# Aster32/GAN-DANet

Measured on AMD Instinct MI355X. Metric: train samples/sec (G+D step) on 256x256 tiles, higher is better.
Workload: dtype bf16; 1 GPU; full G+D train step, 8ch 256x256 -> 1024x1024 tiles, batch 32/GPU (global 32), perceptual=on, SSIM evaluated, AdamW x2; survey_config=3, per_gpu_batch=32, global_batch=32, tile=256, parallelism=dp1

## Files before the change

### gan-danet_amd/csrc/pam.hip

```cpp
#include <stdlib.h>
#include <type_traits>

#include "pam_common.h"
#include "../../include/gandanet.h"

namespace {

using namespace pam;

__device__ __forceinline__ f32x16_t mfma_bf16(bf16x8_t a, bf16x8_t b, f32x16_t c) { return mfma16<false>(a, b, c); }
__device__ __forceinline__ bf16x8_t pack_frag(const f32x16_t& a, int s) { return pam::pack_frag<false>(a, s); }

constexpr int F_KLD = 40;

constexpr int D_KROWCH = 5;

template <int CT, int NW, int KT, bool ONES, bool F16>
__global__ __launch_bounds__(NW * 64, 2) void pam_fwd_dma_kernel(const unsigned short* __restrict__ qt,
                                                            const unsigned short* __restrict__ kt,
                                                            const unsigned short* __restrict__ v, int N, int Npad, int C,
                                                            const float* __restrict__ gamma, const float* __restrict__ x,
                                                            long x_bs, float* __restrict__ out, long out_bs,
                                                            float* __restrict__ o_attn, float* __restrict__ lse,
                                                            const float* __restrict__ k_sqmax,
                                                            const float* __restrict__ mshift, int* __restrict__ redo) {
    if (redo && !mshift && redo[blockIdx.y * gridDim.x + blockIdx.x] == 0) return;
    constexpr int CP = CT * 32;
    constexpr int NSUB = KT / 32;
    constexpr int VROWCH = KT / 8 + 1;
    constexpr int VLD = KT + 8;
    constexpr int KCH = KT * D_KROWCH;
    constexpr int NCH = KCH + CP * VROWCH;
    constexpr int NPIECE = (NCH + 63) / 64;
    constexpr int PPW = (NPIECE + NW - 1) / NW;
    constexpr int TILE = NPIECE * 64 * 8;
    __shared__ __attribute__((aligned(16))) unsigned short ring[2 * TILE];

    const int tid = threadIdx.x, lane = tid & 63, wave = tid >> 6;
    const int r = lane & 31, h = lane >> 5;
    const int b = blockIdx.y;
    const int q0 = blockIdx.x * (NW * 32) + wave * 32;
    const unsigned short* ktb = kt + (long)b * Npad * 32;
    const unsigned short* vb = v + (long)b * CP * Npad;

    bf16x8_t qf[2];
#pragma unroll
    for (int s = 0; s < 2; ++s)
        qf[s] = *reinterpret_cast<const bf16x8_t*>(qt + ((long)b * Npad + q0 + r) * 32 + s * 16 + 8 * h);

    static_assert(KCH % 64 == 0, "a DMA piece must be all-K or all-V");
    unsigned int voff[PPW];
#pragma unroll
    for (int i = 0; i < PPW; ++i) {
        const int piece = wave + NW * i;
        const int c = piece * 64 + lane;
        if (piece * 64 < KCH) {
            const int row = c / D_KROWCH, part = c - row * D_KROWCH;
            voff[i] = (unsigned int)(row * 32 + (part < 4 ? part : 3) * 8) * 2u;
        } else {
            const int c2 = (c < NCH ? c : NCH - 1) - KCH;
            const int row = c2 / VROWCH, part = c2 - row * VROWCH;
            voff[i] = ((unsigned int)row * (unsigned int)Npad + (unsigned int)(part < KT / 8 ? part : KT / 8 - 1) * 8u) * 2u;
        }
    }
    auto dma_tile = [&](int t, int slot) {
        const char* kbase = reinterpret_cast<const char*>(ktb + (long)t * (KT * 32));
        const char* vbase = reinterpret_cast<const char*>(vb + (long)t * KT);
#pragma unroll
        for (int i = 0; i < PPW; ++i) {
            const int piece = wave + NW * i;
            if (piece < NPIECE && piece * 64 + lane < NCH) {
                unsigned short* dst = ring + slot * TILE + piece * 512;
                const char* base = piece * 64 < KCH ? kbase : vbase;
                __builtin_amdgcn_global_load_lds((const __attribute__((address_space(1))) void*)(base + voff[i]),
                                                 (__attribute__((address_space(3))) void*)dst, 16, 0, 0);
            }
        }
    };

    f32x16_t o[CT];
#pragma unroll
    for (int ct = 0; ct < CT; ++ct)
#pragma unroll
        for (int e = 0; e < 16; ++e) o[ct][e] = 0.f;
    float m = 0.f, l = 0.f;
    const int nkt = (N + KT - 1) / KT;

    dma_tile(0, 0);
    auto sweep = [&](auto nm) {
    constexpr bool NOMAX = decltype(nm)::value;
    for (int t = 0; t < nkt; ++t) {
        asm volatile("s_waitcnt vmcnt(0)" ::: "memory");
        __syncthreads();
        if (t + 1 < nkt) dma_tile(t + 1, (t + 1) & 1);
        const unsigned short* Ks = ring + (t & 1) * TILE;
        const unsigned short* Vs = Ks + KCH * 8;

        f32x16_t sacc[NSUB];
#pragma unroll
        for (int sub = 0; sub < NSUB; ++sub) {
#pragma unroll
            for (int e = 0; e < 16; ++e) sacc[sub][e] = 0.f;
#pragma unroll
            for (int s = 0; s < 2; ++s) {
                const bf16x8_t kf = *reinterpret_cast<const bf16x8_t*>(Ks + (sub * 32 + r) * F_KLD + s * 16 + 8 * h);
                sacc[sub] = mfma16<F16>(kf, qf[s], sacc[sub]);
            }
        }
        if ((t + 1) * KT > N) {
#pragma unroll
            for (int sub = 0; sub < NSUB; ++sub)
#pragma unroll
                for (int e = 0; e < 16; ++e)
                    if ((t * KT + sub * 32 + acc_row(e, h)) >= N) sacc[sub][e] = -1e30f;
        }
        float mloc = sacc[0][0];
        if constexpr (!NOMAX) {
#pragma unroll
            for (int sub = 0; sub < NSUB; ++sub)
#pragma unroll
                for (int e = 0; e < 16; ++e) mloc = fmaxf(mloc, sacc[sub][e]);
            mloc = fmaxf(mloc, __shfl_xor(mloc, 32, 64));
        }
        float lsum = 0.f;
        bf16x8_t pf[NSUB][2];
        if (!NOMAX && (t == 0 || __any(mloc > 0.f))) {
            const float want = m + (t == 0 ? mloc : fmaxf(mloc, 0.f));
            float m_new;
            unsigned short m_neg16;
            if constexpr (F16) {
                _Float16 hm = (_Float16)want;
                unsigned short hb = __builtin_bit_cast(unsigned short, hm);
                if ((float)hm < want) hb = (hb & 0x8000u) ? (unsigned short)(hb - 1) : (unsigned short)(hb + 1);
                m_new = (float)__builtin_bit_cast(_Float16, hb);
                m_neg16 = hb ^ 0x8000u;
            } else {
                const unsigned int wb = __builtin_bit_cast(unsigned int, want);
                m_new = __builtin_bit_cast(float, want > 0.f ? (wb + 0xFFFFu) & 0xFFFF0000u : wb & 0xFFFF0000u);
                m_neg16 = (unsigned short)(__builtin_bit_cast(unsigned int, -m_new) >> 16);
            }
            const float shift = m_new - m;
            if (t != 0) {
                const float alpha = gd_exp2_fast(-shift);
                l *= alpha;
#pragma unroll
                for (int ct = 0; ct < CT; ++ct)
#pragma unroll
                    for (int e = 0; e < 16; ++e) o[ct][e] *= alpha;
            }
            m = m_new;
            if (h) qf[1][7] = (short)m_neg16;
#pragma unroll
            for (int sub = 0; sub < NSUB; ++sub) {
#pragma unroll
                for (int e = 0; e < 16; ++e) {
                    sacc[sub][e] = gd_exp2_fast(sacc[sub][e] - shift);
                    if (!ONES) lsum += sacc[sub][e];
                }
                pf[sub][0] = pam::pack_frag<F16>(sacc[sub], 0);
                pf[sub][1] = pam::pack_frag<F16>(sacc[sub], 1);
            }
        } else {
#pragma unroll
            for (int sub = 0; sub < NSUB; ++sub) {
#pragma unroll
                for (int e = 0; e < 16; ++e) {
                    sacc[sub][e] = gd_exp2_fast(sacc[sub][e]);
                    if (!ONES) lsum += sacc[sub][e];
                }
                pf[sub][0] = pam::pack_frag<F16>(sacc[sub], 0);
                pf[sub][1] = pam::pack_frag<F16>(sacc[sub], 1);
            }
        }
        if (!ONES) {
            lsum += __shfl_xor(lsum, 32, 64);
            l += lsum;
        }

#pragma unroll
        for (int ks = 0; ks < 2 * NSUB; ++ks) {
            const int sub = ks >> 1, s2 = ks & 1;
            bf16x8_t vf[CT];
#pragma unroll
            for (int ct = 0; ct < CT; ++ct)
                vf[ct] = *reinterpret_cast<const bf16x8_t*>(Vs + (ct * 32 + r) * VLD + sub * 32 + s2 * 16 + 8 * h);
            __builtin_amdgcn_sched_group_barrier(0x100, CT, 0);
#pragma unroll
            for (int ct = 0; ct < CT; ++ct) o[ct] = mfma16<F16>(vf[ct], pf[sub][s2], o[ct]);
            __builtin_amdgcn_sched_group_barrier(0x008, CT, 0);
        }
    }
    };
    bool nomax = false;
    if (mshift) {
        float mv = mshift[(long)b * Npad + q0 + r];
        m = mv;
        if (h) qf[1][7] = (short)(__builtin_bit_cast(unsigned int, -mv) >> 16);
        nomax = true;
    } else if (k_sqmax) {
        float q2 = 0.f;
#pragma unroll
        for (int s = 0; s < 2; ++s)
#pragma unroll
            for (int e = 0; e < 8; ++e) {
                const float qv = F16 ? (float)__builtin_bit_cast(_Float16, (unsigned short)qf[s][e]) : gd_bf2f((unsigned short)qf[s][e]);
                q2 = fmaf(qv, qv, q2);
            }
        q2 += __shfl_xor(q2, 32, 64);
        const float bound = sqrtf(q2 * k_sqmax[b]) * 1.0001f;
        nomax = __syncthreads_and(bound <= (F16 ? 13.f : 60.f)) != 0;
    }
    if (nomax) sweep(std::true_type{});
    else sweep(std::false_type{});

    if (ONES) l = __shfl(o[CT - 1][15], r + 32, 64);
    if (mshift) {
        const bool bad = !(l > 1e-30f && l < 1e30f) && (q0 + r) < N;
        if (__syncthreads_or(bad) && tid == 0) redo[blockIdx.y * gridDim.x + blockIdx.x] = 1;
    }
    const int qi = q0 + r;
    if (qi < N) {
        const float inv_l = 1.f / l;
        const float g = *gamma;
#pragma unroll
        for (int ct = 0; ct < CT; ++ct)
#pragma unroll
            for (int e = 0; e < 16; ++e) {
                const int c = ct * 32 + acc_row(e, h);
                if (c < C) {
                    const float val = o[ct][e] * inv_l;
                    o_attn[((long)b * C + c) * N + qi] = val;
                    out[(long)b * out_bs + (long)c * N + qi] = fmaf(g, val, x[(long)b * x_bs + (long)c * N + qi]);
                }
            }
        if (h == 0) lse[(long)b * N + qi] = (m + log2f(l)) * LN2;
    }
}


template <int NS, bool F16>
__global__ __launch_bounds__(256) void pam_row_shift_kernel(const unsigned short* __restrict__ qt,
                                                           const unsigned short* __restrict__ kt, int N, int Npad,
                                                           float* __restrict__ mshift) {
    __shared__ __attribute__((aligned(16))) unsigned short ks[NS * 32];
    const int b = blockIdx.y, tid = threadIdx.x;
    const long nb = (long)b * Npad;
    const int stride = N / NS > 0 ? N / NS : 1;
    for (int c = tid; c < NS * 4; c += 256) {
        const int j = c >> 2, part = c & 3;
        const long key = (long)j * stride < N ? (long)j * stride : (long)N - 1;
        *reinterpret_cast<u32x4_t*>(ks + j * 32 + part * 8) = *reinterpret_cast<const u32x4_t*>(kt + (nb + key) * 32 + part * 8);
    }
    __syncthreads();
    const int i = blockIdx.x * 256 + tid;
    if (i >= Npad) return;
    float q[32];
    {
        const u32x4_t* qp = reinterpret_cast<const u32x4_t*>(qt + (nb + i) * 32);
#pragma unroll
        for (int c = 0; c < 4; ++c) {
            const u32x4_t w = qp[c];
#pragma unroll
            for (int e = 0; e < 4; ++e) {
                q[c * 8 + 2 * e] = pam::unpack_lo<F16>(w[e]);
                q[c * 8 + 2 * e + 1] = pam::unpack_hi<F16>(w[e]);
            }
        }
        q[31] = 0.f;
    }
    float best = -3.0e38f;
    for (int j = 0; j < NS; ++j) {
        const u32x4_t* kp = reinterpret_cast<const u32x4_t*>(ks + j * 32);
        float d = 0.f;
#pragma unroll
        for (int c = 0; c < 4; ++c) {
            const u32x4_t w = kp[c];
#pragma unroll
            for (int e = 0; e < 4; ++e) {
                d = fmaf(q[c * 8 + 2 * e], pam::unpack_lo<F16>(w[e]), d);
                d = fmaf(q[c * 8 + 2 * e + 1], pam::unpack_hi<F16>(w[e]), d);
            }
        }
        best = fmaxf(best, d);
    }
    const unsigned int wb = __builtin_bit_cast(unsigned int, best);
    const float up = __builtin_bit_cast(float, best > 0.f ? (wb + 0xFFFFu) & 0xFFFF0000u : wb & 0xFFFF0000u);
    mshift[nb + i] = up;
}

template <int CT, bool DQ, int NW = 4>
__global__ __launch_bounds__(NW * 64, NW == 4 ? 2 : 1) void pam_bwd_dkv3_kernel(
    const unsigned short* __restrict__ qt, const unsigned short* __restrict__ kt, const unsigned short* __restrict__ kn,
    const unsigned short* __restrict__ vt, const unsigned short* __restrict__ dot_, const float* __restrict__ lse,
    const float* __restrict__ delta, int N, int Npad, float* __restrict__ dkn, float* __restrict__ dv,
    unsigned short* __restrict__ dq_part) {
    constexpr int CP = CT * 32;
    constexpr int NT = NW * 64, KEYS = NW * 32;
    constexpr int DLD = CP + 8;
    constexpr int NCHUNK = 128 + 128 * CT;
    constexpr int NPRE = (NCHUNK + NT - 1) / NT;
    constexpr bool RAGGED = (NCHUNK % NT) != 0;
    __shared__ __attribute__((aligned(16))) unsigned short Vls[KEYS * DLD];
    __shared__ __attribute__((aligned(16))) unsigned short Qs[32 * B_QLD];
    constexpr int DOLD = CP + 32;
    __shared__ __attribute__((aligned(16))) unsigned short dOs[32 * DOLD];
    __shared__ float Ls[32], Ds[32];
    constexpr int XLD = 36;
    __shared__ __attribute__((aligned(16))) unsigned short Xs[DQ ? NW * 32 * XLD : 8];

    const int tid = threadIdx.x, lane = tid & 63, wave = tid >> 6;
    const int r = lane & 31, h = lane >> 5;
    const int b = blockIdx.y;
    const int j0 = blockIdx.x * KEYS + wave * 32;
    const long nb = (long)b * Npad;

    bf16x8_t kfB[2];
#pragma unroll
    for (int s = 0; s < 2; ++s) kfB[s] = *reinterpret_cast<const bf16x8_t*>(kt + (nb + j0 + r) * 32 + s * 16 + 8 * h);
    bf16x8_t knA[2];
    if (DQ) {
#pragma unroll
        for (int s = 0; s < 2; ++s)
            knA[s] = *reinterpret_cast<const bf16x8_t*>(kn + ((long)b * 32 + r) * Npad + j0 + s * 16 + 8 * h);
    }
    unsigned short* Xw = Xs + (DQ ? wave * 32 * XLD : 0);
    unsigned short* part = DQ ? dq_part + ((long)b * (Npad / KEYS) + blockIdx.x) * Npad * 32 : nullptr;
    {
        const unsigned short* vsrc = vt + (nb + (long)blockIdx.x * KEYS) * CP;
        for (int c = tid; c < KEYS * (CP / 8); c += NT) {
            const int row = c / (CP / 8), ch = c - row * (CP / 8);
            *reinterpret_cast<u32x4_t*>(Vls + row * DLD + ch * 8) =
                *reinterpret_cast<const u32x4_t*>(vsrc + (long)row * CP + ch * 8);
        }
    }

    f32x16_t dvacc[CT], dkacc;
#pragma unroll
    for (int e = 0; e < 16; ++e) dkacc[e] = 0.f;
#pragma unroll
    for (int ct = 0; ct < CT; ++ct)
#pragma unroll
        for (int e = 0; e < 16; ++e) dvacc[ct][e] = 0.f;

    const bool key_ok = (j0 + r) < N;
// ... 453 lines not shown
```

### gan-danet_amd/csrc/conv3x3.hip

```cpp
#include "common.h"
#include "tile_mma.h"
#include "../../include/gandanet.h"

namespace {

using gd::acc_row;
using gd::bf16x8_native_t;
typedef unsigned int u32x4_t __attribute__((ext_vector_type(4)));

constexpr int TW = 32;
constexpr int PW = TW + 2;
constexpr int CK = 32;
constexpr int LD = CK + 8;

__global__ void pack_w_kernel(const float* __restrict__ a, long a_sm, long a_sc, long a_st, int M, int Ck, int flip,
                              int BM, int nchunks, unsigned short* __restrict__ wp, long total) {
    for (long i = (long)blockIdx.x * blockDim.x + threadIdx.x; i < total; i += (long)gridDim.x * blockDim.x) {
        const int cc = (int)(i % CK);
        long t = i / CK;
        const int mm = (int)(t % BM);
        t /= BM;
        const int tap = (int)(t % 9);
        t /= 9;
        const int chunk = (int)(t % nchunks);
// ... 602 lines not shown
            const long pbase = (((long)b * a.H + Y) * a.W + X) * (a.split ? 3 * a.K : a.K);
#pragma unroll
            for (int g = 0; g < 4; ++g) {
                const int m = mt * BM + wm * 32 + 8 * g + 4 * h;
                if (m >= a.K) continue;
                float v[4];
#pragma unroll
                for (int k = 0; k < 4; ++k) v[k] = acc[c][j][4 * g + k];
                if (a.act) {
                    const uint2 mk = *reinterpret_cast<const uint2*>(a.act + pbase + m);
                    if (!((mk.x & 0x7FFFu) && !(mk.x & 0x8000u))) v[0] *= a.slope;
                    if (!((mk.x >> 16) & 0x7FFFu) || (mk.x >> 31)) v[1] *= a.slope;
                    if (!((mk.y & 0x7FFFu) && !(mk.y & 0x8000u))) v[2] *= a.slope;
                    if (!((mk.y >> 16) & 0x7FFFu) || (mk.y >> 31)) v[3] *= a.slope;
                }
                uint2 o;
                if (a.split) {
                    uint2 lo;
                    gd_split_bf2(v[0], v[1], o.x, lo.x);
                    gd_split_bf2(v[2], v[3], o.y, lo.y);
                    *reinterpret_cast<uint2*>(a.dx + pbase + a.K + m) = lo;
                    *reinterpret_cast<uint2*>(a.dx + pbase + 2 * a.K + m) = o;
                } else {
                    o.x = gd_pack_bf2(v[0], v[1]);
                    o.y = gd_pack_bf2(v[2], v[3]);
                }
                *reinterpret_cast<uint2*>(a.dx + pbase + m) = o;
            }
        }
    }
}

}

extern "C" int gd_conv3x3_nhwc_pack(const float* w, int Cout, int Cin, int transposed, void* ws, size_t ws_bytes,
                                    void* stream) {
    GD_CHECK_ARG(w && ws && Cout > 0 && Cin > 0 && transposed >= 0 && transposed <= 2, "gd_conv3x3_nhwc_pack: bad arguments");
    const int M = transposed ? Cin : Cout, K = transposed ? Cout : Cin;
    GD_CHECK_ARG(ws_bytes >= gd_conv3x3_ws_bytes(M, K), "gd_conv3x3_nhwc_pack: workspace too small");
    const int bm = transposed == 2 ? 64 : pick_bm(M, K);
    const int mtiles = (M + bm - 1) / bm, nchunks = (K + CK - 1) / CK;
    const long total = (long)mtiles * nchunks * 9 * bm * CK;
    int blocks = (int)((total + 255) / 256);
    if (blocks > 2048) blocks = 2048;
    const long sm = transposed ? 9 : (long)Cin * 9, sc = transposed ? (long)Cin * 9 : 9;
    hipLaunchKernelGGL(pack_w_kernel, dim3(blocks), dim3(256), 0, (hipStream_t)stream, w, sm, sc, 1L, M, K,
                       transposed == 1 ? 1 : 0, bm, nchunks, (unsigned short*)ws, total);
    GD_LAUNCH_CHECK();
    return 0;
}

static int nhwc_conv_launch(const void* x, const void* wpack, const float* bias, const void* mask, const void* res,
                            void* y, int B, int H, int W, int K, int M, int stride, int act, float slope, void* stream,
                            float* y32 = nullptr, long y32_bs = 0, int osplit = 0) {
    NhwcConvArgs a;
    static const int epi_env = getenv("GD_NHWC_EPI_LDS") ? atoi(getenv("GD_NHWC_EPI_LDS")) : 1;
    a.y32 = y32; a.y32_bs = y32_bs; a.osplit = osplit; a.epi_lds = epi_env;
    a.x = (const unsigned short*)x; a.wp = (const unsigned short*)wpack; a.bias = bias;
    a.mask = (const unsigned short*)mask; a.res = (const unsigned short*)res; a.y = (unsigned short*)y;
    a.H = H; a.W = W; a.K = K; a.M = M; a.act = act; a.slope = slope;
    a.Ho = (H - 1) / stride + 1; a.Wo = (W - 1) / stride + 1;
    const int bm = pick_bm(M, K);
    const int mtiles = (M + bm - 1) / bm;
    a.nchunks = (K + CK - 1) / CK;
    a.tiles_x = (a.Wo + TW - 1) / TW;
    const int th = stride == 1 ? 8 : 4;
    const int tiles_y = (a.Ho + th - 1) / th;
    dim3 grid(a.tiles_x * tiles_y, mtiles, B);
    hipStream_t s = (hipStream_t)stream;
    if (!a.y32 && a.epi_lds) {
        if (stride == 1) {
            if (bm == 64) hipLaunchKernelGGL((conv3x3_nhwc_kernel<64, 1, 1>), grid, dim3(256), 0, s, a);
            else hipLaunchKernelGGL((conv3x3_nhwc_kernel<128, 1, 1>), grid, dim3(256), 0, s, a);
        } else {
            if (bm == 64) hipLaunchKernelGGL((conv3x3_nhwc_kernel<64, 2, 1>), grid, dim3(256), 0, s, a);
            else hipLaunchKernelGGL((conv3x3_nhwc_kernel<128, 2, 1>), grid, dim3(256), 0, s, a);
        }
    } else if (stride == 1) {
        if (bm == 64) hipLaunchKernelGGL((conv3x3_nhwc_kernel<64, 1>), grid, dim3(256), 0, s, a);
        else hipLaunchKernelGGL((conv3x3_nhwc_kernel<128, 1>), grid, dim3(256), 0, s, a);
    } else {
        if (bm == 64) hipLaunchKernelGGL((conv3x3_nhwc_kernel<64, 2>), grid, dim3(256), 0, s, a);
        else hipLaunchKernelGGL((conv3x3_nhwc_kernel<128, 2>), grid, dim3(256), 0, s, a);
    }
    GD_LAUNCH_CHECK();
    return 0;
}

extern "C" int gd_conv3x3_nhwc(const void* x, const void* wpack, const float* bias, const void* mask, const void* res,
                               void* y, int B, int H, int W, int K, int M, int relu, int split, void* stream) {
    GD_CHECK_ARG(x && wpack && y, "gd_conv3x3_nhwc: null pointer");
    GD_CHECK_ARG(B > 0 && B <= 65535 && H > 0 && W > 0 && K > 0 && M > 0 && K % 8 == 0 && M % 8 == 0,
                 "gd_conv3x3_nhwc: channel counts must be multiples of 8");
    GD_CHECK_ARG((long)H * W * K < (1L << 31) && (long)H * W * M * (split ? 3 : 1) < (1L << 31), "gd_conv3x3_nhwc: image too large");
    return nhwc_conv_launch(x, wpack, bias, mask, res, y, B, H, W, K, M, 1, relu ? 1 : 0, 0.f, stream, nullptr, 0, split ? 1 : 0);
}

extern "C" int gd_conv3x3_nhwc_f32out(const void* x, const void* wpack, const float* bias, float* y32, long y_bs, int B, int H,
                                      int W, int K, int M, int relu, void* stream) {
    GD_CHECK_ARG(x && wpack && y32, "gd_conv3x3_nhwc_f32out: null pointer");
    GD_CHECK_ARG(B > 0 && B <= 65535 && H > 0 && W > 0 && K > 0 && M > 0 && K % 8 == 0 && M % 4 == 0 && y_bs >= (long)M * H * W,
                 "gd_conv3x3_nhwc_f32out: K must be a multiple of 8, M of 4");
    GD_CHECK_ARG((long)H * W * K < (1L << 31), "gd_conv3x3_nhwc_f32out: image too large");
    return nhwc_conv_launch(x, wpack, bias, nullptr, nullptr, nullptr, B, H, W, K, M, 1, relu ? 1 : 0, 0.f, stream, y32, y_bs);
}

extern "C" int gd_conv3x3_nhwc_s2(const void* x, const void* wpack, const float* bias, void* y, int B, int H, int W, int K,
                                  int M, int act, float slope, int split, void* stream) {
    GD_CHECK_ARG(x && wpack && y, "gd_conv3x3_nhwc_s2: null pointer");
    GD_CHECK_ARG(B > 0 && B <= 65535 && H > 0 && W > 0 && K > 0 && M > 0 && K % 8 == 0 && M % 8 == 0 && act >= 0 && act <= 2,
                 "gd_conv3x3_nhwc_s2: channel counts must be multiples of 8, act in 0..2");
    GD_CHECK_ARG((long)H * W * K < (1L << 31) && (long)H * W * M * (split ? 3 : 1) < (1L << 31), "gd_conv3x3_nhwc_s2: image too large");
    return nhwc_conv_launch(x, wpack, bias, nullptr, nullptr, y, B, H, W, K, M, 2, act, slope, stream, nullptr, 0, split ? 1 : 0);
}

extern "C" int gd_conv3x3_nhwc_s2_dgrad(const void* dy, const void* wpack_t, const void* act_out, float slope, void* dx,
                                        int B, int H, int W, int K, int M, int split, void* stream) {
    GD_CHECK_ARG(dy && wpack_t && dx, "gd_conv3x3_nhwc_s2_dgrad: null pointer");
    GD_CHECK_ARG(B > 0 && B <= 65535 && H > 0 && W > 0 && K > 0 && M > 0 && K % 8 == 0 && M % 8 == 0,
                 "gd_conv3x3_nhwc_s2_dgrad: channel counts must be multiples of 8");
    GD_CHECK_ARG((long)H * W * K * (split ? 3 : 1) < (1L << 31) && (long)H * W * M < (1L << 31), "gd_conv3x3_nhwc_s2_dgrad: image too large");
    NhwcDgrad2Args a;
    a.split = split ? 1 : 0;
    a.dy = (const unsigned short*)dy; a.wp = (const unsigned short*)wpack_t; a.act = (const unsigned short*)act_out;
    a.dx = (unsigned short*)dx; a.H = H; a.W = W; a.K = K; a.M = M; a.slope = slope;
    a.Ho = (H - 1) / 2 + 1; a.Wo = (W - 1) / 2 + 1;
    a.nchunks = (M + CK - 1) / CK;
    a.tiles_x = (a.Wo + TW - 1) / TW;
    const int tiles_y = (a.Ho + 3) / 4;
    dim3 grid(a.tiles_x * tiles_y, (K + 63) / 64, B);
    hipLaunchKernelGGL(conv3x3_nhwc_dgrad2_kernel, grid, dim3(256), 0, (hipStream_t)stream, a);
    GD_LAUNCH_CHECK();
    return 0;
}

namespace {

typedef short s16x4_t __attribute__((ext_vector_type(4)));
constexpr int WTH = 4;
constexpr int WPH = WTH + 2;
constexpr int WNPIX = WPH * PW;
constexpr int DYLD = WTH * TW + 8;

struct WgradArgs {
    const unsigned short* dy16;
    const float* dy; long dy_bs;
    const float* x; long x_bs;
    const unsigned short* x16; int x16_ld;
    const float* in_scale; const float* in_shift; int in_relu;
    float* dw;
    float* part;
    int B, M, Ck, H, W, Ho, Wo;
    int tiles_x, tiles_y, tiles_per_split;
};
typedef float f32x4u_t __attribute__((ext_vector_type(4), aligned(4)));

__device__ __forceinline__ s16x4_t lds_tr_read(const unsigned short* p) {
    return __builtin_amdgcn_ds_read_tr16_b64_v4i16((__attribute__((address_space(3))) s16x4_t*)p);
}

#ifndef GD_WGRAD_PIPED_MINW
#define GD_WGRAD_PIPED_MINW 1
#endif
template <int NW, int S, bool CS, bool PIPED = false, bool ORD = false>
__global__ __launch_bounds__(NW * 64, PIPED ? GD_WGRAD_PIPED_MINW : 2) void conv3x3_wgrad_kernel(const WgradArgs a) {
    constexpr int BM = CS ? 32 : 32 * NW, NT = 64 * NW, NCH = CS ? NW : 1;
    constexpr int PHk = S * (WTH - 1) + 3, PWk = S * (TW - 1) + 3, NPIXk = PHk * PWk;
    __shared__ __attribute__((aligned(16))) unsigned short dys[BM * DYLD];
    __shared__ __attribute__((aligned(16))) unsigned short patch[NCH * NPIXk * LD];

    const int tid = threadIdx.x, lane = tid & 63, wave = tid >> 6;
    const int r = lane & 31, h = lane >> 5;
    const int c0 = blockIdx.x * CK * NCH;
    const int m0 = blockIdx.y * BM;
    const long HW = (long)a.H * a.W;
    const long HWo = (long)a.Ho * a.Wo;
    const int ntiles = a.B * a.tiles_y * a.tiles_x;
    const int t_begin = blockIdx.z * a.tiles_per_split;
    const int t_end = min(ntiles, t_begin + a.tiles_per_split);

    f32x16_t acc[9];
#pragma unroll
    for (int t = 0; t < 9; ++t)
#pragma unroll
        for (int e = 0; e < 16; ++e) acc[t][e] = 0.f;

    const int li = lane & 15, tq = li >> 2, tp = li & 3, tg = (lane >> 4) & 1;
    const bool vec_ok = (a.Wo % 4) == 0;

    constexpr bool piped = PIPED;
    constexpr int NDY = PIPED ? (BM * 32 + NT - 1) / NT : 1;
    constexpr int NXI = PIPED ? (4 * NCH * NPIXk + NT - 1) / NT : 1;
    uint2 rdy[NDY];
    u32x4_t rxp[NXI];
    auto load_regs = [&](int t) {
        const int b = t / (a.tiles_y * a.tiles_x);
        const int rem = t - b * (a.tiles_y * a.tiles_x);
        const int ty_ = rem / a.tiles_x, tx_ = rem - ty_ * a.tiles_x;
        const int y0 = ty_ * WTH, x0 = tx_ * TW;
#pragma unroll
        for (int k = 0; k < NDY; ++k) {
            const int idx = tid + k * NT;
            const int m = idx >> 5, v = idx & 31;
            const int yy = y0 + (v >> 3), xx = x0 + (v & 7) * 4;
            uint2 w = make_uint2(0u, 0u);
            if (idx < BM * 32 && m0 + m < a.M && yy < a.Ho) {
                const unsigned short* p = a.dy16 + ((long)b * a.M + m0 + m) * HWo + (long)yy * a.Wo + xx;
                if (vec_ok && xx + 3 < a.Wo) {
                    w = *reinterpret_cast<const uint2*>(p);
                } else {
                    unsigned int e0 = xx + 0 < a.Wo ? p[0] : 0u, e1 = xx + 1 < a.Wo ? p[1] : 0u;
                    unsigned int e2 = xx + 2 < a.Wo ? p[2] : 0u, e3 = xx + 3 < a.Wo ? p[3] : 0u;
                    w.x = e0 | (e1 << 16);
                    w.y = e2 | (e3 << 16);
                }
            }
            rdy[k] = w;
        }
#pragma unroll
        for (int k = 0; k < NXI; ++k) {
            const int w = tid + k * NT;
            const int oc = w / NPIXk;
            const int q = oc & 3, chk = oc >> 2;
            const int pix = w - oc * NPIXk;
            const int py = pix / PWk, px = pix - py * PWk;
            const int iy = S * y0 - 1 + py, ix = S * x0 - 1 + px;
            const int cb = c0 + chk * CK + q * 8;
            u32x4_t v = {0u, 0u, 0u, 0u};
            if (w < 4 * NCH * NPIXk && iy >= 0 && iy < a.H && ix >= 0 && ix < a.W && cb < a.x16_ld)
                v = *reinterpret_cast<const u32x4_t*>(a.x16 + (((long)b * a.H + iy) * a.W + ix) * a.x16_ld + cb);
            rxp[k] = v;
        }
    };
    auto store_regs = [&]() {
#pragma unroll
        for (int k = 0; k < NDY; ++k) {
            const int idx = tid + k * NT;
            if (idx < BM * 32) *reinterpret_cast<uint2*>(dys + (idx >> 5) * DYLD + (idx & 31) * 4) = rdy[k];
        }
#pragma unroll
        for (int k = 0; k < NXI; ++k) {
            const int w = tid + k * NT;
            if (w < 4 * NCH * NPIXk) {
                const int oc = w / NPIXk;
                const int pix = w - oc * NPIXk;
                *reinterpret_cast<u32x4_t*>(patch + ((oc >> 2) * NPIXk + pix) * LD + (oc & 3) * 8) = rxp[k];
            }
        }
    };
    if constexpr (piped) {
        if (t_begin < t_end) load_regs(t_begin);
    }

    for (int t = t_begin; t < t_end; ++t) {
        const int b = t / (a.tiles_y * a.tiles_x);
        const int rem = t - b * (a.tiles_y * a.tiles_x);
        const int ty_ = rem / a.tiles_x, tx_ = rem - ty_ * a.tiles_x;
        const int y0 = ty_ * WTH, x0 = tx_ * TW;
        const float* dyb = a.dy + (long)b * a.dy_bs;
        const float* xb = a.x + (long)b * a.x_bs;

        if constexpr (piped) {
            store_regs();
        } else {
#pragma unroll 4
        for (int k = 0; k < 16 / (CS ? NW : 1) + (CS && (16 % NW) ? 1 : 0); ++k) {
            const int idx = tid + k * NT;
            if (CS && idx >= 32 * 32) break;
            const int m = idx >> 5, v = idx & 31;
            const int yy = y0 + (v >> 3), xx = x0 + (v & 7) * 4;
            if (a.dy16) {
                uint2 w = make_uint2(0u, 0u);
                if (m0 + m < a.M && yy < a.Ho) {
                    const unsigned short* p = a.dy16 + ((long)b * a.M + m0 + m) * HWo + (long)yy * a.Wo + xx;
                    if (vec_ok && xx + 3 < a.Wo) {
                        w = *reinterpret_cast<const uint2*>(p);
                    } else {
                        unsigned int e0 = xx + 0 < a.Wo ? p[0] : 0u, e1 = xx + 1 < a.Wo ? p[1] : 0u;
                        unsigned int e2 = xx + 2 < a.Wo ? p[2] : 0u, e3 = xx + 3 < a.Wo ? p[3] : 0u;
                        w.x = e0 | (e1 << 16);
                        w.y = e2 | (e3 << 16);
                    }
                }
                *reinterpret_cast<uint2*>(dys + m * DYLD + v * 4) = w;
                continue;
            }
            float4 f = make_float4(0.f, 0.f, 0.f, 0.f);
            if (m0 + m < a.M && yy < a.Ho) {
                const float* p = dyb + (long)(m0 + m) * HWo + (long)yy * a.Wo + xx;
                if (vec_ok && xx + 3 < a.Wo) {
                    f = *reinterpret_cast<const float4*>(p);
                } else {
                    if (xx + 0 < a.Wo) f.x = p[0];
                    if (xx + 1 < a.Wo) f.y = p[1];
                    if (xx + 2 < a.Wo) f.z = p[2];
                    if (xx + 3 < a.Wo) f.w = p[3];
                }
            }
            uint2 w;
            w.x = gd_pack_bf2(f.x, f.y);
            w.y = gd_pack_bf2(f.z, f.w);
            *reinterpret_cast<uint2*>(dys + m * DYLD + v * 4) = w;
        }
        if (a.x16) {
            for (int w = tid; w < 4 * NCH * NPIXk; w += NT) {
                const int oc = w / NPIXk;
                const int q = oc & 3, chk = oc >> 2;
                const int pix = w - oc * NPIXk;
                const int py = pix / PWk, px = pix - py * PWk;
                const int iy = S * y0 - 1 + py, ix = S * x0 - 1 + px;
                const int cb = c0 + chk * CK + q * 8;
                u32x4_t v = {0u, 0u, 0u, 0u};
                if (iy >= 0 && iy < a.H && ix >= 0 && ix < a.W && cb < a.x16_ld)
                    v = *reinterpret_cast<const u32x4_t*>(a.x16 + (((long)b * a.H + iy) * a.W + ix) * a.x16_ld + cb);
                *reinterpret_cast<u32x4_t*>(patch + (chk * NPIXk + pix) * LD + q * 8) = v;
            }
        } else
        for (int w = tid; w < 2 * NCH * NPIXk; w += NT) {
            const int hc = w / NPIXk;
            const int half = hc & 1, chk = hc >> 1;
            const int pix = w - hc * NPIXk;
            const int py = pix / PWk, px = pix - py * PWk;
            const int iy = S * y0 - 1 + py, ix = S * x0 - 1 + px;
            const bool inside = iy >= 0 && iy < a.H && ix >= 0 && ix < a.W;
            const int cb = c0 + chk * CK + half * 16;
            const float* p = xb + (long)cb * HW + (long)iy * a.W + ix;
            unsigned int* dst = reinterpret_cast<unsigned int*>(patch + (chk * NPIXk + pix) * LD + half * 16);
#pragma unroll
            for (int j = 0; j < 8; ++j) {
                const int c = cb + 2 * j;
                float v0 = 0.f, v1 = 0.f;
                if (inside) {
                    if (c < a.Ck) v0 = p[(long)(2 * j) * HW];
                    if (c + 1 < a.Ck) v1 = p[(long)(2 * j + 1) * HW];
                    if (a.in_scale) {
                        if (c < a.Ck) {
                            v0 = fmaf(v0, a.in_scale[c], a.in_shift[c]);
                            if (a.in_relu) v0 = fmaxf(v0, 0.f);
                        }
                        if (c + 1 < a.Ck) {
                            v1 = fmaf(v1, a.in_scale[c + 1], a.in_shift[c + 1]);
                            if (a.in_relu) v1 = fmaxf(v1, 0.f);
                        }
                    }
                }
                dst[j] = gd_pack_bf2(v0, v1);
            }
        }
        }
        __syncthreads();
        if constexpr (piped) {
            if (t + 1 < t_end) load_regs(t + 1);
        }

#pragma unroll 2
        for (int s = 0; s < 8; ++s) {
            const bf16x8_t fa = *reinterpret_cast<const bf16x8_t*>(dys + ((CS ? 0 : wave * 32) + r) * DYLD + 16 * s + 8 * h);
            const int prow = s >> 1, pcol = (s & 1) * 16 + 8 * h + tq;
#pragma unroll
            for (int ky = 0; ky < 3; ++ky)
#pragma unroll
                for (int kx = 0; kx < 3; ++kx) {
                    const unsigned short* p0 = patch + ((CS ? wave * NPIXk : 0) + (prow * S + ky) * PWk + pcol * S + kx) * LD +
                                               16 * tg + 4 * tp;
                    const s16x4_t lo = lds_tr_read(p0);
                    const s16x4_t hi = lds_tr_read(p0 + 4 * S * LD);
                    const bf16x8_t fb = {lo.x, lo.y, lo.z, lo.w, hi.x, hi.y, hi.z, hi.w};
                    acc[ky * 3 + kx] = __builtin_amdgcn_mfma_f32_32x32x16_bf16(
                        __builtin_bit_cast(bf16x8_native_t, fa), __builtin_bit_cast(bf16x8_native_t, fb),
                        acc[ky * 3 + kx], 0, 0, 0);
                }
        }
        __syncthreads();
    }

    const int ci = c0 + (CS ? wave * CK : 0) + r;
    if constexpr (ORD) {
        if (ci < a.Ck) {
            float* pw = a.part + (long)blockIdx.z * a.M * a.Ck * 9;
#pragma unroll
            for (int e = 0; e < 16; ++e) {
                const int co = m0 + (CS ? 0 : wave * 32) + acc_row(e, h);
                if (co < a.M) {
                    float* q = pw + ((long)co * a.Ck + ci) * 9;
                    const f32x4u_t v0 = {acc[0][e], acc[1][e], acc[2][e], acc[3][e]};
                    const f32x4u_t v1 = {acc[4][e], acc[5][e], acc[6][e], acc[7][e]};
                    *reinterpret_cast<f32x4u_t*>(q) = v0;
                    *reinterpret_cast<f32x4u_t*>(q + 4) = v1;
                    q[8] = acc[8][e];
                }
            }
        }
    } else if (ci < a.Ck) {
#pragma unroll
        for (int t = 0; t < 9; ++t)
#pragma unroll
            for (int e = 0; e < 16; ++e) {
                const int co = m0 + (CS ? 0 : wave * 32) + acc_row(e, h);
                if (co < a.M) atomicAdd(a.dw + ((long)co * a.Ck + ci) * 9 + t, acc[t][e]);
            }
    }
}

}

static const bool g_wgrad_cs_piped = getenv("GD_WGRAD_CS_PIPED") ? atoi(getenv("GD_WGRAD_CS_PIPED")) != 0 : true;
static const bool g_wgrad_s2_piped = getenv("GD_WGRAD_S2_PIPED") ? atoi(getenv("GD_WGRAD_S2_PIPED")) != 0 : true;

namespace {
struct WgradPlan {
    int best_nw, cs, groups, cs_nw, mblocks, tiles_x, tiles_y, Ho, Wo, tiles_per_split, splits, ordered;
    long ntiles;
    size_t ws_needed;
};
int wgrad_plan(int B, int Cout, int Cin, int H, int W, int stride, size_t ws_bytes, WgradPlan* p) {
    GD_CHECK_ARG(B > 0 && Cout > 0 && Cin > 0 && H > 0 && W > 0 && (stride == 1 || stride == 2), "gd_conv3x3_wgrad: bad sizes");
    p->Ho = (H - 1) / stride + 1; p->Wo = (W - 1) / stride + 1;
    p->tiles_x = (p->Wo + TW - 1) / TW;
    p->tiles_y = (p->Ho + WTH - 1) / WTH;
    const long ntiles = (long)B * p->tiles_x * p->tiles_y;
    GD_CHECK_ARG(ntiles < (1L << 31), "gd_conv3x3_wgrad: too many tiles");
    p->ntiles = ntiles;
    int best_nw = 2;
    long best_pad = -1;
    for (int nw : {2, 4, 6}) {
        const long bm = 32L * nw, pad = ((Cout + bm - 1) / bm) * bm;
        if (best_pad < 0 || pad <= best_pad) { best_pad = pad; best_nw = nw; }
    }
    const int chunks = (Cin + CK - 1) / CK;
    const bool cs = Cout <= 32 && stride == 1 && chunks >= 3;
    const int groups = cs ? (chunks + 3) / 4 : chunks;
    const int cs_nw = cs ? (chunks + groups - 1) / groups : 0;
    const int bm = cs ? 32 : 32 * best_nw;
    const int mblocks = (Cout + bm - 1) / bm;
    p->best_nw = best_nw; p->cs = cs; p->groups = groups; p->cs_nw = cs_nw; p->mblocks = mblocks;
    const bool det = gd_get_deterministic() != 0, ordered_mode = det && gd_get_det_reduce() == 1;
    long splits = 1024 / ((long)mblocks * groups);
    if (splits < 1 || (det && !ordered_mode)) splits = 1;
    if (splits > ntiles) splits = ntiles;
    if (splits > 65535) splits = 65535;
    const size_t out_bytes = (size_t)Cout * Cin * 9 * sizeof(float);
    if (ordered_mode) {
        const size_t fit = ws_bytes / out_bytes;
        if ((size_t)splits > fit) splits = (long)fit;
        if (splits < 2) splits = 1;
    }
    p->tiles_per_split = (int)((ntiles + splits - 1) / splits);
    splits = (ntiles + p->tiles_per_split - 1) / p->tiles_per_split;
    p->splits = (int)splits;
    p->ordered = ordered_mode && splits > 1;
    p->ws_needed = p->ordered ? (size_t)splits * out_bytes : 0;
    return 0;
}
}

extern "C" int gd_conv3x3_wgrad_plan(int B, int Cout, int Cin, int H, int W, int stride, size_t ws_bytes, int* splits,
                                     size_t* ws_needed) {
    WgradPlan p;
    if (wgrad_plan(B, Cout, Cin, H, W, stride, ws_bytes, &p)) return -1;
    if (splits) *splits = p.splits;
    if (ws_needed) *ws_needed = p.ws_needed;
    return 0;
}

extern "C" int gd_conv3x3_wgrad_ws(const float* dy, long dy_bs, const void* dy_bf16, const float* x, long x_bs,
                                   const void* x_nhwc16, int x_ld, const float* in_scale, const float* in_shift, int in_relu,
                                   int B, int Cout, int Cin, int H, int W, int stride, int accumulate, float* dw, void* stream,
                                   void* ws, size_t ws_bytes) {
    GD_CHECK_ARG((dy || dy_bf16) && (x || x_nhwc16) && dw, "gd_conv3x3_wgrad: null pointer");
    GD_CHECK_ARG(!x_nhwc16 || (!in_scale && x_ld >= Cin && x_ld % 8 == 0),
                 "gd_conv3x3_wgrad: the pixel-major bf16 x needs x_ld >= Cin, x_ld % 8 == 0 and no input transform");
    GD_CHECK_ARG((in_scale == nullptr) == (in_shift == nullptr), "gd_conv3x3_wgrad: in_scale/in_shift must come together");
    GD_CHECK_ARG(((uintptr_t)ws % 16) == 0, "gd_conv3x3_wgrad: the workspace must be 16-byte aligned");
    WgradPlan p;
    if (wgrad_plan(B, Cout, Cin, H, W, stride, ws ? ws_bytes : 0, &p)) return -1;
    hipStream_t s = (hipStream_t)stream;
    if (!accumulate && !p.ordered)
        GD_CHECK_ARG(hipMemsetAsync(dw, 0, (size_t)Cout * Cin * 9 * sizeof(float), s) == hipSuccess, "gd_conv3x3_wgrad: memset failed");
    WgradArgs a;
    a.dy16 = (const unsigned short*)dy_bf16;
    a.dy = dy; a.dy_bs = dy_bs; a.x = x; a.x_bs = x_bs;
    a.x16 = (const unsigned short*)x_nhwc16; a.x16_ld = x_ld;
    a.in_scale = in_scale; a.in_shift = in_shift; a.in_relu = in_relu;
    a.dw = dw; a.part = p.ordered ? (float*)ws : nullptr;
    a.B = B; a.M = Cout; a.Ck = Cin; a.H = H; a.W = W;
    a.Ho = p.Ho; a.Wo = p.Wo; a.tiles_x = p.tiles_x; a.tiles_y = p.tiles_y;
    a.tiles_per_split = p.tiles_per_split;
    const int best_nw = p.best_nw, cs_nw = p.cs_nw, groups = p.groups, mblocks = p.mblocks, splits = p.splits;
    const bool cs = p.cs != 0;
    dim3 grid(groups, mblocks, (unsigned)splits);
#define WG_LAUNCH(NW_, S_, CS_, PIPED_, THREADS_)                                                                             \
    do {                                                                                                                      \
        if (p.ordered) hipLaunchKernelGGL((conv3x3_wgrad_kernel<NW_, S_, CS_, PIPED_, true>), grid, dim3(THREADS_), 0, s, a); \
        else hipLaunchKernelGGL((conv3x3_wgrad_kernel<NW_, S_, CS_, PIPED_, false>), grid, dim3(THREADS_), 0, s, a);          \
    } while (0)
    if (cs && a.dy16 && a.x16 && g_wgrad_cs_piped) {
        if (cs_nw == 3) WG_LAUNCH(3, 1, true, true, 192);
        else WG_LAUNCH(4, 1, true, true, 256);
    } else if (cs) {
        if (cs_nw == 3) WG_LAUNCH(3, 1, true, false, 192);
        else WG_LAUNCH(4, 1, true, false, 256);
    } else if (stride == 1 && a.dy16 && a.x16 && best_nw >= 4) {
        if (best_nw == 4) WG_LAUNCH(4, 1, false, true, 256);
        else WG_LAUNCH(6, 1, false, true, 384);
    } else if (stride == 1) {
        if (best_nw == 2) WG_LAUNCH(2, 1, false, false, 128);
        else if (best_nw == 4) WG_LAUNCH(4, 1, false, false, 256);
        else WG_LAUNCH(6, 1, false, false, 384);
    } else if (a.dy16 && a.x16 && best_nw == 4 && g_wgrad_s2_piped) {
        WG_LAUNCH(4, 2, false, true, 256);
    } else {
        if (best_nw == 2) WG_LAUNCH(2, 2, false, false, 128);
        else if (best_nw == 4) WG_LAUNCH(4, 2, false, false, 256);
        else WG_LAUNCH(6, 2, false, false, 384);
    }
#undef WG_LAUNCH
    GD_LAUNCH_CHECK();
    if (p.ordered) return gd_det_reduce_launch(a.part, splits, dw, 1, 1, Cout * Cin * 9, 0, (long)Cout * Cin * 9, nullptr, accumulate, s);
    return 0;
}

extern "C" int gd_conv3x3_wgrad(const float* dy, long dy_bs, const void* dy_bf16, const float* x, long x_bs,
                                const void* x_nhwc16, int x_ld, const float* in_scale, const float* in_shift, int in_relu,
                                int B, int Cout, int Cin, int H, int W, int stride, int accumulate, float* dw, void* stream) {
    return gd_conv3x3_wgrad_ws(dy, dy_bs, dy_bf16, x, x_bs, x_nhwc16, x_ld, in_scale, in_shift, in_relu, B, Cout, Cin, H, W, stride,
                               accumulate, dw, stream, nullptr, 0);
}
```

Before: 38.02 samples/s.

## Split PAM forward DMA into K and V phases with counted vmcnt waits

Splits the per-tile global-to-LDS DMA into separate K and V parts. Half the waves are staggered so the K and V loads for upcoming tiles are issued at two points per iteration, and partial s_waitcnt vmcnt counts are used instead of draining all loads. It also replaces the builtin LDS DMA with inline asm that sets m0 from a scalar (readfirstlane) address, so wave-uniform values stay in scalar registers. The aim is better overlap of memory loads with the QK and PV MFMA phases. It adds an extra barrier per iteration and a fragile hand-counted wait scheme that could race if the counts are wrong.

Result: no change. 38.19 samples/s, median of 6 (+0.4%).

```diff
diff --git a/gan-danet_amd/csrc/pam.hip b/gan-danet_amd/csrc/pam.hip
--- a/gan-danet_amd/csrc/pam.hip
+++ b/gan-danet_amd/csrc/pam.hip
@@ -12,6 +12,19 @@
 __device__ __forceinline__ bf16x8_t pack_frag(const f32x16_t& a, int s) { return pam::pack_frag<false>(a, s); }
 
 constexpr int F_KLD = 40;
+
+template <int N>
+__device__ __forceinline__ void wait_vmcnt() { asm volatile("s_waitcnt vmcnt(%0)" ::"n"(N) : "memory"); }
+
+constexpr int dma_min_pieces(int nw, int i0, int lo, int hi) {
+    int best = 1 << 30;
+    for (int w = 0; w < nw; ++w) {
+        int n = 0;
+        for (int p = w + nw * i0; p < hi; p += nw) n += p >= lo;
+        best = n < best ? n : best;
+    }
+    return best;
+}
 
 constexpr int D_KROWCH = 5;
 
@@ -36,7 +49,8 @@
     constexpr int TILE = NPIECE * 64 * 8;
     __shared__ __attribute__((aligned(16))) unsigned short ring[2 * TILE];
 
-    const int tid = threadIdx.x, lane = tid & 63, wave = tid >> 6;
+    const int tid = threadIdx.x, lane = tid & 63;
+    const int wave = __builtin_amdgcn_readfirstlane(tid >> 6);
     const int r = lane & 31, h = lane >> 5;
     const int b = blockIdx.y;
     const int q0 = blockIdx.x * (NW * 32) + wave * 32;
@@ -63,17 +77,21 @@
             voff[i] = ((unsigned int)row * (unsigned int)Npad + (unsigned int)(part < KT / 8 ? part : KT / 8 - 1) * 8u) * 2u;
         }
     }
-    auto dma_tile = [&](int t, int slot) {
+    constexpr int NKP = KCH / 64;
+    constexpr int KMIN = dma_min_pieces(NW, 0, 0, NKP), VMIN = dma_min_pieces(NW, 0, NKP, NPIECE);
+    static_assert(KMIN >= 1 && VMIN >= 1 && VMIN < 64, "counted DMA waits: every wave issues at least one piece per batch");
+    const unsigned int ring_lds = (unsigned int)(size_t)(__attribute__((address_space(3))) unsigned short*)ring;
+    auto dma_part = [&](int t, int slot, bool kpart) {
         const char* kbase = reinterpret_cast<const char*>(ktb + (long)t * (KT * 32));
         const char* vbase = reinterpret_cast<const char*>(vb + (long)t * KT);
 #pragma unroll
         for (int i = 0; i < PPW; ++i) {
             const int piece = wave + NW * i;
-            if (piece < NPIECE && piece * 64 + lane < NCH) {
-                unsigned short* dst = ring + slot * TILE + piece * 512;
-                const char* base = piece * 64 < KCH ? kbase : vbase;
-                __builtin_amdgcn_global_load_lds((const __attribute__((address_space(1))) void*)(base + voff[i]),
-                                                 (__attribute__((address_space(3))) void*)dst, 16, 0, 0);
+            if ((piece < NKP) == kpart && piece < NPIECE && piece * 64 + lane < NCH) {
+                const unsigned int dst = __builtin_amdgcn_readfirstlane(ring_lds + (slot * TILE + piece * 512) * 2);
+                const char* base = piece < NKP ? kbase : vbase;
+                asm volatile("s_mov_b32 m0, %0\n\ts_nop 0\n\tglobal_load_lds_dwordx4 %1, %2" ::"s"(dst), "v"(voff[i]), "s"(base)
+                             : "memory");
             }
         }
     };
@@ -86,13 +104,26 @@
     float m = 0.f, l = 0.f;
     const int nkt = (N + KT - 1) / KT;
 
-    dma_tile(0, 0);
+    dma_part(0, 0, true);
+    dma_part(0, 0, false);
+    const bool late = wave >= NW / 2;
+    int pend = VMIN;
+    auto next_interval = [&](bool kpart, int tn) {
+        if (pend == 0) wait_vmcnt<0>();
+        else if (pend == KMIN) wait_vmcnt<KMIN>();
+        else wait_vmcnt<VMIN>();
+        __syncthreads();
+        pend = 0;
+        if (tn < nkt) {
+            dma_part(tn, tn & 1, kpart);
+            pend = kpart ? KMIN : VMIN;
+        }
+    };
     auto sweep = [&](auto nm) {
     constexpr bool NOMAX = decltype(nm)::value;
+    if (late) next_interval(true, 1);
     for (int t = 0; t < nkt; ++t) {
-        asm volatile("s_waitcnt vmcnt(0)" ::: "memory");
-        __syncthreads();
-        if (t + 1 < nkt) dma_tile(t + 1, (t + 1) & 1);
+        next_interval(!late, t + 1);
         const unsigned short* Ks = ring + (t & 1) * TILE;
         const unsigned short* Vs = Ks + KCH * 8;
 
@@ -177,6 +208,8 @@
             l += lsum;
         }
 
+        next_interval(late, late ? t + 2 : t + 1);
+
 #pragma unroll
         for (int ks = 0; ks < 2 * NSUB; ++ks) {
             const int sub = ks >> 1, s2 = ks & 1;
@@ -190,6 +223,7 @@
             __builtin_amdgcn_sched_group_barrier(0x008, CT, 0);
         }
     }
+    if (!late) next_interval(true, nkt);
     };
     bool nomax = false;
     if (mshift) {
```

## Add ky-split blocked wgrad kernel with double-buffered LDS and XCD-aware grid remap

Applied to the files above, without the earlier changes.

Adds a new 3x3 weight-gradient kernel for the stride-1 bf16 piped path. Six waves split work by kernel row (ky) and output-channel group, and each wave holds MT*3 accumulators across kx taps. The kernel double-buffers the dy and input-patch tiles in LDS, prefetching the next tile in phases while the MFMAs run. Workgroups are remapped so consecutive logical blocks land on the same XCD, aiming for better L2 reuse. In exchange it uses more LDS and registers (launch bounds 384 threads with min 1 block), which lowers occupancy, and its weight layout writes strided kx outputs.

Result: no change. 38.01 samples/s before, 38.18 samples/s after (median of 6 runs) (+0.4%).

```diff
diff --git a/gan-danet_amd/csrc/conv3x3.hip b/gan-danet_amd/csrc/conv3x3.hip
--- a/gan-danet_amd/csrc/conv3x3.hip
+++ b/gan-danet_amd/csrc/conv3x3.hip
@@ -778,6 +778,7 @@
     float* part;
     int B, M, Ck, H, W, Ho, Wo;
     int tiles_x, tiles_y, tiles_per_split;
+    int groups, mblocks, splits, wg_per_xcd;
 };
 typedef float f32x4u_t __attribute__((ext_vector_type(4), aligned(4)));
 
@@ -1026,6 +1027,168 @@
                 if (co < a.M) atomicAdd(a.dw + ((long)co * a.Ck + ci) * 9 + t, acc[t][e]);
             }
     }
+}
+
+
+template <int MT, bool ORD>
+__global__ __launch_bounds__(384, 1) void conv3x3_wgrad_blocked_kernel(const WgradArgs a) {
+    constexpr int BM = 64 * MT, NT = 384;
+    __shared__ __attribute__((aligned(16))) unsigned short dys[2][BM * DYLD];
+    __shared__ __attribute__((aligned(16))) unsigned short patch[2][WNPIX * LD];
+
+    const int wg = (blockIdx.x & 7) * a.wg_per_xcd + (blockIdx.x >> 3);
+    if (wg >= a.groups * a.mblocks * a.splits) return;
+    const int grp = wg % a.groups, mb = (wg / a.groups) % a.mblocks, split = wg / (a.groups * a.mblocks);
+
+    const int tid = threadIdx.x, lane = tid & 63, wave = tid >> 6;
+    const int r = lane & 31, h = lane >> 5;
+    const int ky = wave % 3, mg = wave / 3;
+    const int c0 = grp * CK;
+    const int m0 = mb * BM;
+    const long HWo = (long)a.Ho * a.Wo;
+    const int ntiles = a.B * a.tiles_y * a.tiles_x;
+    const int t_begin = split * a.tiles_per_split;
+    const int t_end = min(ntiles, t_begin + a.tiles_per_split);
+
+    f32x16_t acc[MT * 3];
+#pragma unroll
+    for (int t = 0; t < MT * 3; ++t)
+#pragma unroll
+        for (int e = 0; e < 16; ++e) acc[t][e] = 0.f;
+
+    const int li = lane & 15, tq = li >> 2, tp = li & 3, tg = (lane >> 4) & 1;
+    const bool vec_ok = (a.Wo % 4) == 0;
+
+    constexpr int NDY = (BM * 32 + NT - 1) / NT;
+    constexpr int NPH = 4, NDYH = (NDY + NPH - 1) / NPH;
+    static_assert((4 * WNPIX + NT - 1) / NT <= NPH, "one patch item per phase");
+    constexpr int NXI = (4 * WNPIX + NT - 1) / NT;
+    uint2 rdy[NDYH];
+    u32x4_t rxp;
+    auto load_dy = [&](int t, int half) {
+        const int b = t / (a.tiles_y * a.tiles_x);
+        const int rem = t - b * (a.tiles_y * a.tiles_x);
+        const int ty_ = rem / a.tiles_x, tx_ = rem - ty_ * a.tiles_x;
+        const int y0 = ty_ * WTH, x0 = tx_ * TW;
+#pragma unroll
+        for (int k = 0; k < NDYH; ++k) {
+            const int idx = tid + (half * NDYH + k) * NT;
+            const int m = idx >> 5, v = idx & 31;
+            const int yy = y0 + (v >> 3), xx = x0 + (v & 7) * 4;
+            uint2 w = make_uint2(0u, 0u);
+            if (idx < BM * 32 && m0 + m < a.M && yy < a.Ho) {
+                const unsigned short* p = a.dy16 + ((long)b * a.M + m0 + m) * HWo + (long)yy * a.Wo + xx;
+                if (vec_ok && xx + 3 < a.Wo) {
+                    w = *reinterpret_cast<const uint2*>(p);
+                } else {
+                    unsigned int e0 = xx + 0 < a.Wo ? p[0] : 0u, e1 = xx + 1 < a.Wo ? p[1] : 0u;
+                    unsigned int e2 = xx + 2 < a.Wo ? p[2] : 0u, e3 = xx + 3 < a.Wo ? p[3] : 0u;
+                    w.x = e0 | (e1 << 16);
+                    w.y = e2 | (e3 << 16);
+                }
+            }
+            rdy[k] = w;
+        }
+    };
+    auto load_patch = [&](int t, int k) {
+        const int b = t / (a.tiles_y * a.tiles_x);
+        const int rem = t - b * (a.tiles_y * a.tiles_x);
+        const int ty_ = rem / a.tiles_x, tx_ = rem - ty_ * a.tiles_x;
+        const int y0 = ty_ * WTH, x0 = tx_ * TW;
+        {
+            const int w = tid + k * NT;
+            const int q = w / WNPIX;
+            const int pix = w - q * WNPIX;
+            const int py = pix / PW, px = pix - py * PW;
+            const int iy = y0 - 1 + py, ix = x0 - 1 + px;
+            const int cb = c0 + q * 8;
+            u32x4_t v = {0u, 0u, 0u, 0u};
+            if (w < 4 * WNPIX && iy >= 0 && iy < a.H && ix >= 0 && ix < a.W && cb < a.x16_ld)
+                v = *reinterpret_cast<const u32x4_t*>(a.x16 + (((long)b * a.H + iy) * a.W + ix) * a.x16_ld + cb);
+            rxp = v;
+        }
+    };
+    auto store_dy = [&](int buf, int half) {
+#pragma unroll
+        for (int k = 0; k < NDYH; ++k) {
+            const int idx = tid + (half * NDYH + k) * NT;
+            if (idx < BM * 32) *reinterpret_cast<uint2*>(dys[buf] + (idx >> 5) * DYLD + (idx & 31) * 4) = rdy[k];
+        }
+    };
+    auto store_patch = [&](int buf, int k) {
+        {
+            const int w = tid + k * NT;
+            if (w < 4 * WNPIX) {
+                const int q = w / WNPIX;
+                *reinterpret_cast<u32x4_t*>(patch[buf] + (w - q * WNPIX) * LD + q * 8) = rxp;
+            }
+        }
+    };
+    if (t_begin < t_end) {
+#pragma unroll
+        for (int ph = 0; ph < NPH; ++ph) {
+            load_dy(t_begin, ph);
+            if (ph < NXI) load_patch(t_begin, ph);
+            store_dy(0, ph);
+            if (ph < NXI) store_patch(0, ph);
+        }
+    }
+    __syncthreads();
+
+    for (int t = t_begin; t < t_end; ++t) {
+        const int cur = (t - t_begin) & 1;
+        const bool more = t + 1 < t_end;
+        const unsigned short* dyw = dys[cur] + (mg * MT * 32 + r) * DYLD + 8 * h;
+        const unsigned short* pw = patch[cur] + (ky * PW + 8 * h + tq) * LD + 16 * tg + 4 * tp;
+#pragma unroll
+        for (int ph = 0; ph < NPH; ++ph) {
+            if (more) {
+                load_dy(t + 1, ph);
+                if (ph < NXI) load_patch(t + 1, ph);
+            }
+#pragma unroll
+            for (int s = 2 * ph; s < 2 * ph + 2; ++s) {
+                bf16x8_t fa[MT];
+#pragma unroll
+                for (int i = 0; i < MT; ++i) fa[i] = *reinterpret_cast<const bf16x8_t*>(dyw + i * 32 * DYLD + 16 * s);
+                const unsigned short* ps = pw + ((s >> 1) * PW + (s & 1) * 16) * LD;
+#pragma unroll
+                for (int kx = 0; kx < 3; ++kx) {
+                    const s16x4_t lo = lds_tr_read(ps + kx * LD);
+                    const s16x4_t hi = lds_tr_read(ps + (kx + 4) * LD);
+                    const bf16x8_t fb = {lo.x, lo.y, lo.z, lo.w, hi.x, hi.y, hi.z, hi.w};
+#pragma unroll
+                    for (int i = 0; i < MT; ++i)
+                        acc[i * 3 + kx] = __builtin_amdgcn_mfma_f32_32x32x16_bf16(
+                            __builtin_bit_cast(bf16x8_native_t, fa[i]), __builtin_bit_cast(bf16x8_native_t, fb),
+                            acc[i * 3 + kx], 0, 0, 0);
+                }
+            }
+            if (more) {
+                store_dy(cur ^ 1, ph);
+                if (ph < NXI) store_patch(cur ^ 1, ph);
+            }
+        }
+        __syncthreads();
+    }
+
+    const int ci = c0 + r;
+    if (ci >= a.Ck) return;
+    float* out = ORD ? a.part + (long)split * a.M * a.Ck * 9 : a.dw;
+#pragma unroll
+    for (int i = 0; i < MT; ++i)
+#pragma unroll
+        for (int e = 0; e < 16; ++e) {
+            const int co = m0 + (mg * MT + i) * 32 + acc_row(e, h);
+            if (co < a.M) {
+                float* q = out + ((long)co * a.Ck + ci) * 9 + ky * 3;
+#pragma unroll
+                for (int kx = 0; kx < 3; ++kx) {
+                    if constexpr (ORD) q[kx] = acc[i * 3 + kx][e];
+                    else atomicAdd(q + kx, acc[i * 3 + kx][e]);
+                }
+            }
+        }
 }
 
 }
@@ -1127,8 +1290,16 @@
         if (cs_nw == 3) WG_LAUNCH(3, 1, true, false, 192);
         else WG_LAUNCH(4, 1, true, false, 256);
     } else if (stride == 1 && a.dy16 && a.x16 && best_nw >= 4) {
-        if (best_nw == 4) WG_LAUNCH(4, 1, false, true, 256);
-        else WG_LAUNCH(6, 1, false, true, 384);
+        const long nwg = (long)groups * mblocks * splits;
+        a.groups = groups; a.mblocks = mblocks; a.splits = splits; a.wg_per_xcd = (int)((nwg + 7) / 8);
+        const dim3 bgrid(8u * a.wg_per_xcd);
+        if (best_nw == 4) {
+            if (p.ordered) hipLaunchKernelGGL((conv3x3_wgrad_blocked_kernel<2, true>), bgrid, dim3(384), 0, s, a);
+            else hipLaunchKernelGGL((conv3x3_wgrad_blocked_kernel<2, false>), bgrid, dim3(384), 0, s, a);
+        } else {
+            if (p.ordered) hipLaunchKernelGGL((conv3x3_wgrad_blocked_kernel<3, true>), bgrid, dim3(384), 0, s, a);
+            else hipLaunchKernelGGL((conv3x3_wgrad_blocked_kernel<3, false>), bgrid, dim3(384), 0, s, a);
+        }
     } else if (stride == 1) {
         if (best_nw == 2) WG_LAUNCH(2, 1, false, false, 128);
         else if (best_nw == 4) WG_LAUNCH(4, 1, false, false, 256);
```
